# Y-Claw/Multilevel-GNN

Measured on AMD Instinct MI355X. Metric: graphs/sec fwd+bwd, 3-level GNN on 10k-node d=128 synthetic; HBM GB/s %peak, higher is better.
Workload: dtype f32; 1 GPU; configs[1]: ER graphs N=10000 E=160000 x64 per GPU, d=128, 3 GENConv(softmax, res+, LayerNorm) + projection pooling G=25000 k=2 + DiffPool 146->37->10, fp32; step = CSR build (of the next batch, on a second stream) + fwd + bwd + grad all-reduce + Adam; graphs_per_gpu=64, global_batch=64, parallelism=dp1, world_size=1, allreduce_bytes=1429768

## Files before the change

multilevel-gnn_amd/csrc/densesage.hip:

```cpp
#include "common.h"
#include "launch.h"
#include "mlgnn.h"
#include "tile_gemm.h"

namespace mlgnn {

constexpr int kDsMaxN = 160, kDsMaxC = 128, kDsMaxO = 64, kDsMaxNAdj = 48;
constexpr int kDsBlock = 1024, kDsWaves = kDsBlock / kWave;
constexpr int kDsSO = kDsMaxO + 1;
constexpr float kDsNormEps = 1e-12f;

struct DsArgs {
  const void* x; const void* adj; const void* w_rel; const void* w_root; const float* bias;
  const void* gy; const void* y; const float* rinv_in;
  void* y_out; float* rinv; void* gx; void* gadj; float* ws;
  int n; int C; int O; int adj_batched; int normalize; int ws_cols;
};

template <typename AB>
__device__ __forceinline__ void ds_degrees(const AB ab, int n, float* deg, float* raw) {
  const int lane = threadIdx.x & (kWave - 1), wave = threadIdx.x / kWave;
  for (int r = wave; r < n; r += kDsWaves) {
    float s = 0.f;
    for (int j = lane; j < n; j += kWave) s += ab[(size_t)r * n + j];
#pragma unroll
    for (int off = 32; off > 0; off >>= 1) s += __shfl_xor(s, off);
    if (lane == 0) {
      if (raw) raw[r] = s;
      deg[r] = fmaxf(s, 1.0f);
    }
  }
}

struct DsLds { int so, sx, np; };
__host__ __device__ inline DsLds ds_lds(int n, int C, int O) {
  DsLds l;
  l.np = (n + 15) & ~15;
  l.so = ((O + 15) & ~15) + 1;
  l.sx = C + 1 + (C & 1);
  return l;
}
inline size_t ds_fwd_lds_bytes(int n, int C, int O) {
  const DsLds l = ds_lds(n, C, O);
  return ((size_t)l.np * l.so + (size_t)l.np * l.sx + l.np) * 4;
}
inline size_t ds_bwd_lds_bytes(int n, int C, int O, bool adj_grad) {
  const DsLds l = ds_lds(n, C, O);
  size_t f = (size_t)2 * l.np * l.so + 2 * l.np;
  if (adj_grad) f += (size_t)l.np * l.so + (size_t)l.np * (l.np + 1);
  return f * 4;
}

template <typename T>
__global__ __launch_bounds__(kDsBlock) void dense_sage_fwd_kernel(const DsArgs p) {
  extern __shared__ __attribute__((aligned(16))) float ds_smem[];
  const int b = blockIdx.x, tid = threadIdx.x;
  const int lane = tid & (kWave - 1), wave = tid / kWave;
  const int n = p.n, C = p.C, O = p.O;
  const DsLds L = ds_lds(n, C, O);
  const int SO = L.so, SX = L.sx;
  float* Pm_ = ds_smem;
  float* Xm_ = Pm_ + (size_t)L.np * SO;
  float* deg = Xm_ + (size_t)L.np * SX;
#define P(r, c) Pm_[(r) * SO + (c)]
#define X(r, c) Xm_[(r) * SX + (c)]
  const StoredIn<T> xb{static_cast<const T*>(p.x) + (size_t)b * n * C};
  const StoredIn<T> ab{static_cast<const T*>(p.adj) + (p.adj_batched ? (size_t)b * n * n : 0)};
  const StoredIn<T> w_rel{static_cast<const T*>(p.w_rel)}, w_root{static_cast<const T*>(p.w_root)};
  const int NP = (n + 15) & ~15, OP = (O + 15) & ~15;
  const int Nt = NP / 16, Ot = OP / 16;
  const int l15 = lane & 15, lq = lane >> 4;

  ds_degrees(ab, n, deg, nullptr);
  for (int idx = tid; idx < NP * C; idx += kDsBlock) {
    const int r = idx / C, c = idx % C;
    X(r, c) = r < n ? xb[idx] : 0.f;
  }
  __syncthreads();
  for (int t = wave; t < Nt * Ot; t += kDsWaves) {
    const int i0 = (t / Ot) * 16, j0 = (t % Ot) * 16;
    const f32x4 acc = tile_gemm(C,
        [&](int i, int k) { return k < C ? X(i0 + i, k) : 0.f; },
        [&](int k, int j) { return (j0 + j < O && k < C) ? w_rel[(size_t)(j0 + j) * C + k] : 0.f; });
#pragma unroll
    for (int r = 0; r < 4; ++r) P(i0 + lq * 4 + r, j0 + l15) = acc[r];
  }
  __syncthreads();
  f32x4 keep[(kDsMaxN / 16) * (kDsMaxO / 16) / kDsWaves + 1];
  int nk = 0;
  for (int t = wave; t < Nt * Ot; t += kDsWaves, ++nk) {
    const int i0 = (t / Ot) * 16, j0 = (t % Ot) * 16;
    f32x4 acc = tile_gemm(n,
        [&](int i, int k) { return (i0 + i < n && k < n) ? ab[(size_t)(i0 + i) * n + k] : 0.f; },
        [&](int k, int j) { return k < n ? P(k, j0 + j) : 0.f; });
    const f32x4 root = tile_gemm(C,
        [&](int i, int k) { return k < C ? X(i0 + i, k) : 0.f; },
        [&](int k, int j) { return (j0 + j < O && k < C) ? w_root[(size_t)(j0 + j) * C + k] : 0.f; });
    const float bj = (p.bias && j0 + l15 < O) ? p.bias[j0 + l15] : 0.f;
#pragma unroll
    for (int r = 0; r < 4; ++r) {
      const int row = i0 + lq * 4 + r;
      acc[r] = acc[r] / deg[min(row, n - 1)] + root[r] + bj;
    }
    keep[nk] = acc;
  }
  __syncthreads();
  nk = 0;
  for (int t = wave; t < Nt * Ot; t += kDsWaves, ++nk) {
    const int i0 = (t / Ot) * 16, j0 = (t % Ot) * 16;
#pragma unroll
    for (int r = 0; r < 4; ++r) P(i0 + lq * 4 + r, j0 + l15) = keep[nk][r];
  }
  __syncthreads();
  for (int r = wave; r < n; r += kDsWaves) {
    const float v = lane < O ? P(r, lane) : 0.f;
    float ss = v * v;
#pragma unroll
    for (int off = 32; off > 0; off >>= 1) ss += __shfl_xor(ss, off);
    const float ri = p.normalize ? 1.0f / fmaxf(sqrtf(ss), kDsNormEps) : 1.0f;
    if (lane < O) stored_write<T>(p.y_out, ((size_t)b * n + r) * O + lane, v * ri);
    if (lane == 0) p.rinv[(size_t)b * n + r] = ri;
  }
}
#undef P
#undef X

template <typename T>
__global__ __launch_bounds__(kDsBlock) void dense_sage_bwd_kernel(const DsArgs p) {
  extern __shared__ __attribute__((aligned(16))) float ds_smem[];
  const int b = blockIdx.x, tid = threadIdx.x;
  const int lane = tid & (kWave - 1), wave = tid / kWave;
  const int n = p.n, C = p.C, O = p.O;
  const DsLds L = ds_lds(n, C, O);
  const int SO = L.so, SM = L.np + 1;
  float* G_ = ds_smem;
  float* GP_ = G_ + (size_t)L.np * SO;
  float* deg = GP_ + (size_t)L.np * SO;
  float* raw = deg + L.np;
  float* Pm_ = raw + L.np;
  float* M_ = Pm_ + (size_t)L.np * SO;
#define G(r, c) G_[(r) * SO + (c)]
#define GP(r, c) GP_[(r) * SO + (c)]
#define Pm(r, c) Pm_[(r) * SO + (c)]
#define M(r, c) M_[(r) * SM + (c)]
  const StoredIn<T> xb{static_cast<const T*>(p.x) + (size_t)b * n * C};
  const StoredIn<T> ab{static_cast<const T*>(p.adj) + (p.adj_batched ? (size_t)b * n * n : 0)};
  const StoredIn<T> w_rel{static_cast<const T*>(p.w_rel)}, w_root{static_cast<const T*>(p.w_root)};
  const StoredIn<T> gyb{static_cast<const T*>(p.gy) + (size_t)b * n * O};
  const StoredIn<T> yb{static_cast<const T*>(p.y) + (size_t)b * n * O};
  const int NP = (n + 15) & ~15, OP = (O + 15) & ~15, CP = (C + 15) & ~15;
  const int Nt = NP / 16, Ot = OP / 16, Ct = CP / 16;
  const int l15 = lane & 15, lq = lane >> 4;

  ds_degrees(ab, n, deg, raw);
  for (int r = wave; r < NP; r += kDsWaves) {
    float gv = 0.f, yv = 0.f;
    if (r < n && lane < O) { gv = gyb[(size_t)r * O + lane]; yv = yb[(size_t)r * O + lane]; }
    float dot = gv * yv;
#pragma unroll
    for (int off = 32; off > 0; off >>= 1) dot += __shfl_xor(dot, off);
    const float ri = r < n ? p.rinv_in[(size_t)b * n + r] : 0.f;
    const float g = p.normalize ? (gv - yv * dot) * ri : gv;
    if (lane < OP) G(r, lane) = (r < n && lane < O) ? g : 0.f;
  }
  __syncthreads();
  for (int t = wave; t < Nt * Ot; t += kDsWaves) {
    const int i0 = (t / Ot) * 16, j0 = (t % Ot) * 16;
    const f32x4 acc = tile_gemm(n,
        [&](int i, int k) { return (i0 + i < n && k < n) ? ab[(size_t)k * n + i0 + i] : 0.f; },
        [&](int k, int j) { return k < n ? G(k, j0 + j) / deg[k] : 0.f; });
#pragma unroll
    for (int r = 0; r < 4; ++r) GP(i0 + lq * 4 + r, j0 + l15) = acc[r];
  }
  __syncthreads();
  const size_t gx_off = (size_t)b * n * C;
  for (int t = wave; t < Nt * Ct; t += kDsWaves) {
    const int i0 = (t / Ct) * 16, c0 = (t % Ct) * 16;
    f32x4 acc = tile_gemm(O,
        [&](int i, int k) { return k < O ? GP(i0 + i, k) : 0.f; },
        [&](int k, int j) { return (k < O && c0 + j < C) ? w_rel[(size_t)k * C + c0 + j] : 0.f; });
    const f32x4 t2 = tile_gemm(O,
        [&](int i, int k) { return k < O ? G(i0 + i, k) : 0.f; },
        [&](int k, int j) { return (k < O && c0 + j < C) ? w_root[(size_t)k * C + c0 + j] : 0.f; });
#pragma unroll
    for (int r = 0; r < 4; ++r) {
      const int row = i0 + lq * 4 + r, col = c0 + l15;
      if (row < n && col < C) stored_write<T>(p.gx, gx_off + (size_t)row * C + col, acc[r] + t2[r]);
    }
  }
  float* wsb = p.ws + (size_t)b * p.ws_cols;
  for (int t = wave; t < 2 * Ot * Ct; t += kDsWaves) {
    const int which = t / (Ot * Ct), tt = t % (Ot * Ct);
    const int o0 = (tt / Ct) * 16, c0 = (tt % Ct) * 16;
    const float* src = which == 0 ? GP_ : G_;
    const f32x4 acc = tile_gemm(n,
        [&](int i, int k) { return k < n ? src[k * SO + o0 + i] : 0.f; },
        [&](int k, int j) { return (k < n && c0 + j < C) ? xb[(size_t)k * C + c0 + j] : 0.f; });
#pragma unroll
    for (int r = 0; r < 4; ++r) {
      const int o = o0 + lq * 4 + r, c = c0 + l15;
      if (o < O && c < C) wsb[(size_t)which * O * C + (size_t)o * C + c] = acc[r];
    }
  }
  for (int o = tid; o < O; o += kDsBlock) {
    float s = 0.f;
    for (int r = 0; r < n; ++r) s += G(r, o);
    wsb[(size_t)2 * O * C + o] = s;
  }
  if (p.gadj) {
    for (int t = wave; t < Nt * Ot; t += kDsWaves) {
      const int i0 = (t / Ot) * 16, j0 = (t % Ot) * 16;
      const f32x4 acc = tile_gemm(C,
          [&](int i, int k) { return (i0 + i < n && k < C) ? xb[(size_t)(i0 + i) * C + k] : 0.f; },
          [&](int k, int j) { return (j0 + j < O && k < C) ? w_rel[(size_t)(j0 + j) * C + k] : 0.f; });
#pragma unroll
      for (int r = 0; r < 4; ++r) Pm(i0 + lq * 4 + r, j0 + l15) = acc[r];
    }
    __syncthreads();
    for (int t = wave; t < Nt * Nt; t += kDsWaves) {
      const int i0 = (t / Nt) * 16, j0 = (t % Nt) * 16;
      const f32x4 acc = tile_gemm(O,
          [&](int i, int k) { return k < O ? G(i0 + i, k) : 0.f; },
          [&](int k, int j) { return k < O ? Pm(j0 + j, k) : 0.f; });
#pragma unroll
      for (int r = 0; r < 4; ++r) M(i0 + lq * 4 + r, j0 + l15) = acc[r];
    }
    __syncthreads();
    const size_t ga_off = (size_t)b * n * n;
    for (int r = wave; r < n; r += kDsWaves) {
      float c = lane < n ? ab[(size_t)r * n + lane] * M(r, lane) : 0.f;
#pragma unroll
      for (int off = 32; off > 0; off >>= 1) c += __shfl_xor(c, off);
      const float ci = raw[r] >= 1.0f ? c / deg[r] : 0.f;
      if (lane < n) stored_write<T>(p.gadj, ga_off + (size_t)r * n + lane, (M(r, lane) - ci) / deg[r]);
    }
  }
}
#undef G
#undef GP
#undef Pm
#undef M

static bool ds_dims_ok(int64_t n, int64_t C, int64_t O) {
  return n >= 1 && n <= kDsMaxN && C >= 1 && C <= kDsMaxC && O >= 1 && O <= kDsMaxO;
}

}

using namespace mlgnn;

extern "C" int mlgnn_dense_sage_supported(int64_t n, int64_t C, int64_t O, int need_grad_adj) {
  return (ds_dims_ok(n, C, O) && (!need_grad_adj || n <= kDsMaxNAdj)) ? 1 : 0;
}

extern "C" int64_t mlgnn_dense_sage_bwd_workspace_floats(int64_t B, int64_t C, int64_t O) {
  if (B < 0 || C <= 0 || O <= 0) return MLGNN_E_SHAPE;
  return B * (2 * O * C + O);
}

extern "C" int mlgnn_dense_sage_fwd(const void* x, const void* adj, const void* w_rel, const void* w_root,
                                    const float* bias, void* y, float* rinv, int64_t B, int64_t n, int64_t C,
                                    int64_t O, int adj_batched, int normalize, int dtype, void* stream) {
  if (dtype != MLGNN_DTYPE_F32 && dtype != MLGNN_DTYPE_BF16) return MLGNN_E_DTYPE;
  if (B < 0 || !ds_dims_ok(n, C, O)) return MLGNN_E_SHAPE;
  if (B == 0) return 0;
  if (!x || !adj || !w_rel || !w_root || !y || !rinv) return MLGNN_E_NULL;
  DsArgs a = {};
  a.x = x; a.adj = adj; a.w_rel = w_rel; a.w_root = w_root;
  a.bias = bias; a.y_out = y; a.rinv = rinv;
  a.n = (int)n; a.C = (int)C; a.O = (int)O; a.adj_batched = adj_batched; a.normalize = normalize;
  const size_t lds = ds_fwd_lds_bytes((int)n, (int)C, (int)O);
  static size_t fwd_attr = 0;
  if (lds > fwd_attr) {
    const int most = (int)ds_fwd_lds_bytes(kDsMaxN, kDsMaxC, kDsMaxO);
    if (const hipError_t e = allow_dynamic_lds(&dense_sage_fwd_kernel<float>, most); e != hipSuccess) return (int)e;
    if (const hipError_t e = allow_dynamic_lds(&dense_sage_fwd_kernel<bf16_t>, most); e != hipSuccess) return (int)e;
    fwd_attr = (size_t)most;
  }
  if (dtype == MLGNN_DTYPE_BF16) hipLaunchKernelGGL(dense_sage_fwd_kernel<bf16_t>, dim3((unsigned)B), dim3(kDsBlock), lds, (hipStream_t)stream, a);
  else hipLaunchKernelGGL(dense_sage_fwd_kernel<float>, dim3((unsigned)B), dim3(kDsBlock), lds, (hipStream_t)stream, a);
  return (int)hipGetLastError();
}

extern "C" int mlgnn_dense_sage_bwd(const void* grad_y, const void* y, const float* rinv, const void* x,
                                    const void* adj, const void* w_rel, const void* w_root, void* grad_x,
                                    void* grad_adj, float* grad_w, float* workspace, int64_t workspace_floats,
                                    int64_t B, int64_t n, int64_t C, int64_t O, int adj_batched, int normalize,
                                    int dtype, void* stream) {
  if (dtype != MLGNN_DTYPE_F32 && dtype != MLGNN_DTYPE_BF16) return MLGNN_E_DTYPE;
  if (B < 0 || !ds_dims_ok(n, C, O)) return MLGNN_E_SHAPE;
  if (grad_adj && n > kDsMaxNAdj) return MLGNN_E_SHAPE;
  if (!grad_w) return MLGNN_E_NULL;
  const int cols = (int)(2 * O * C + O);
  hipStream_t s = (hipStream_t)stream;
  if (B == 0) return (int)hipMemsetAsync(grad_w, 0, (size_t)cols * 4, s);
  if (!grad_y || !y || !rinv || !x || !adj || !w_rel || !w_root || !grad_x || !workspace) return MLGNN_E_NULL;
  if (workspace_floats < B * cols) return MLGNN_E_WORKSPACE;
  DsArgs a = {};
  a.x = x; a.adj = adj; a.w_rel = w_rel; a.w_root = w_root;
  a.gy = grad_y; a.y = y; a.rinv_in = rinv;
  a.gx = grad_x; a.gadj = grad_adj; a.ws = workspace; a.ws_cols = cols;
  a.n = (int)n; a.C = (int)C; a.O = (int)O; a.adj_batched = adj_batched; a.normalize = normalize;
  const size_t lds = ds_bwd_lds_bytes((int)n, (int)C, (int)O, grad_adj != nullptr);
  static size_t bwd_attr = 0;
  if (lds > bwd_attr) {
    const size_t most = ds_bwd_lds_bytes(kDsMaxN, kDsMaxC, kDsMaxO, false) > ds_bwd_lds_bytes(kDsMaxNAdj, kDsMaxC, kDsMaxO, true)
                            ? ds_bwd_lds_bytes(kDsMaxN, kDsMaxC, kDsMaxO, false) : ds_bwd_lds_bytes(kDsMaxNAdj, kDsMaxC, kDsMaxO, true);
    if (const hipError_t e = allow_dynamic_lds(&dense_sage_bwd_kernel<float>, (int)most); e != hipSuccess) return (int)e;
    if (const hipError_t e = allow_dynamic_lds(&dense_sage_bwd_kernel<bf16_t>, (int)most); e != hipSuccess) return (int)e;
    bwd_attr = most;
  }
  if (dtype == MLGNN_DTYPE_BF16) hipLaunchKernelGGL(dense_sage_bwd_kernel<bf16_t>, dim3((unsigned)B), dim3(kDsBlock), lds, s, a);
  else hipLaunchKernelGGL(dense_sage_bwd_kernel<float>, dim3((unsigned)B), dim3(kDsBlock), lds, s, a);
  int err = (int)hipGetLastError();
  if (err) return err;
  launch_reduce_partials(workspace, grad_w, (int)B, cols, s);
  return (int)hipGetLastError();
}
```

multilevel-gnn_amd/csrc/tile_gemm.h:

```cpp
#pragma once
#include "common.h"

namespace mlgnn {

using f32x4 = __attribute__((ext_vector_type(4))) float;

constexpr int kTileUnroll = 8;

template <typename FA, typename FB>
__device__ __forceinline__ f32x4 tile_gemm(int kdim, FA a_at, FB b_at) {
  const int lane = threadIdx.x & (kWave - 1);
  const int l15 = lane & 15, lk = lane >> 4;
  f32x4 acc = {0.f, 0.f, 0.f, 0.f};
  for (int k0 = 0; k0 < kdim; k0 += 4 * kTileUnroll) {
    float a[kTileUnroll], b[kTileUnroll];
#pragma unroll
    for (int u = 0; u < kTileUnroll; ++u) {
      a[u] = a_at(l15, k0 + 4 * u + lk);
      b[u] = b_at(k0 + 4 * u + lk, l15);
    }
#pragma unroll
    for (int u = 0; u < kTileUnroll; ++u) acc = __builtin_amdgcn_mfma_f32_16x16x4f32(a[u], b[u], acc, 0, 0, 0);
  }
  return acc;
}

}
```

Measured before the change: 5505 graphs/s.

## Stage DenseSAGE forward operands in LDS and keep weight fragments register-resident

The dense SAGE forward kernel now stages x, both weight matrices, and the adjacency into LDS using 16-byte vector loads where alignment allows, instead of reading weights and adjacency element-wise from global memory inside the MFMA loops. Each wave owns a fixed column tile and keeps its W_rel/W_root fragments in registers, computing the rel and root products for up to three row tiles in one pass. Degrees are then computed from the LDS copy of the adjacency, and the separate keep/write-back pass is merged into a single epilogue. This cuts redundant global traffic and strided scalar loads, at the cost of higher LDS usage, an extra sync inside the K-block loop, and more register pressure from the resident fragments.

```diff
diff --git a/multilevel-gnn_amd/csrc/densesage.hip b/multilevel-gnn_amd/csrc/densesage.hip
--- a/multilevel-gnn_amd/csrc/densesage.hip
+++ b/multilevel-gnn_amd/csrc/densesage.hip
@@ -7,22 +7,24 @@
 
 constexpr int kDsMaxN = 160, kDsMaxC = 128, kDsMaxO = 64, kDsMaxNAdj = 48;
 constexpr int kDsBlock = 1024, kDsWaves = kDsBlock / kWave;
-constexpr int kDsSO = kDsMaxO + 1;
 constexpr float kDsNormEps = 1e-12f;
+constexpr int kDsFwdTiles = 3;
+static_assert(kDsFwdTiles * (kDsWaves / (kDsMaxO / 16)) >= kDsMaxN / 16, "row tiles of one column tile per wave");
 
 struct DsArgs {
   const void* x; const void* adj; const void* w_rel; const void* w_root; const float* bias;
   const void* gy; const void* y; const float* rinv_in;
   void* y_out; float* rinv; void* gx; void* gadj; float* ws;
   int n; int C; int O; int adj_batched; int normalize; int ws_cols;
+  int vec16;
 };
 
 template <typename AB>
-__device__ __forceinline__ void ds_degrees(const AB ab, int n, float* deg, float* raw) {
+__device__ __forceinline__ void ds_degrees(const AB ab, int n, int stride, float* deg, float* raw) {
   const int lane = threadIdx.x & (kWave - 1), wave = threadIdx.x / kWave;
   for (int r = wave; r < n; r += kDsWaves) {
     float s = 0.f;
-    for (int j = lane; j < n; j += kWave) s += ab[(size_t)r * n + j];
+    for (int j = lane; j < n; j += kWave) s += ab[(size_t)r * stride + j];
 #pragma unroll
     for (int off = 32; off > 0; off >>= 1) s += __shfl_xor(s, off);
     if (lane == 0) {
@@ -32,23 +34,64 @@
   }
 }
 
-struct DsLds { int so, sx, np; };
+struct DsLds { int so, sx, sa, np, op; };
 __host__ __device__ inline DsLds ds_lds(int n, int C, int O) {
   DsLds l;
   l.np = (n + 15) & ~15;
-  l.so = ((O + 15) & ~15) + 1;
-  l.sx = C + 1 + (C & 1);
+  l.op = (O + 15) & ~15;
+  l.so = l.op + 1;
+  l.sx = ((C + 31) & ~31) + 1;
+  l.sa = ((n + 31) & ~31) + 1;
   return l;
+}
+__host__ __device__ inline int ds_fwd_floats(const DsLds& l) {
+  const int first = l.np * l.sx + 2 * l.op * l.sx, then = l.np * (l.sx > l.sa ? l.sx : l.sa) + l.np * l.so;
+  return first > then ? first : then;
 }
 inline size_t ds_fwd_lds_bytes(int n, int C, int O) {
   const DsLds l = ds_lds(n, C, O);
-  return ((size_t)l.np * l.so + (size_t)l.np * l.sx + l.np) * 4;
+  return ((size_t)ds_fwd_floats(l) + l.np) * 4;
 }
 inline size_t ds_bwd_lds_bytes(int n, int C, int O, bool adj_grad) {
   const DsLds l = ds_lds(n, C, O);
   size_t f = (size_t)2 * l.np * l.so + 2 * l.np;
   if (adj_grad) f += (size_t)l.np * l.so + (size_t)l.np * (l.np + 1);
   return f * 4;
+}
+
+template <typename T, int V>
+__device__ __forceinline__ void ds_stage_run(float* img, int stride, const T* src, int cols, int first, int count) {
+  const int step = V * kDsBlock, dr = step / cols, dc = step - dr * cols;
+  int e = first + V * (int)threadIdx.x;
+  int r = e / cols, c = e - r * cols;
+  for (int i = threadIdx.x; i < count; i += kDsBlock, e += step) {
+    float v[V];
+    load_t<T, V>(v, src + e);
+    int rr = r, cc = c;
+#pragma unroll
+    for (int q = 0; q < V; ++q) {
+      img[rr * stride + cc] = v[q];
+      if (++cc == cols) { cc = 0; ++rr; }
+    }
+    c += dc; r += dr;
+    if (c >= cols) { c -= cols; ++r; }
+  }
+}
+
+template <typename T>
+__device__ __forceinline__ void ds_stage(float* img, int stride, const T* src, int rows, int cols, int rows_p,
+                                         int cols_p, int vec16) {
+  constexpr int V = 16 / (int)sizeof(T);
+  const int lane = threadIdx.x & (kWave - 1), wave = threadIdx.x / kWave;
+  const int total = rows * cols;
+  int head = total;
+  if (vec16) head = min(total, (int)(((0 - reinterpret_cast<uintptr_t>(src)) & 15) / sizeof(T)));
+  const int nvec = (total - head) / V;
+  ds_stage_run<T, 1>(img, stride, src, cols, 0, head);
+  if (nvec > 0) ds_stage_run<T, V>(img, stride, src, cols, head, nvec);
+  ds_stage_run<T, 1>(img, stride, src, cols, head + V * nvec, total - head - V * nvec);
+  for (int r = wave; r < rows_p; r += kDsWaves)
+    for (int c = (r < rows ? cols : 0) + lane; c < cols_p; c += kWave) img[r * stride + c] = 0.f;
 }
 
 template <typename T>
@@ -58,58 +101,79 @@
   const int lane = tid & (kWave - 1), wave = tid / kWave;
   const int n = p.n, C = p.C, O = p.O;
   const DsLds L = ds_lds(n, C, O);
-  const int SO = L.so, SX = L.sx;
-  float* Pm_ = ds_smem;
-  float* Xm_ = Pm_ + (size_t)L.np * SO;
-  float* deg = Xm_ + (size_t)L.np * SX;
+  const int SO = L.so, SX = L.sx, SA = L.sa;
+  float* Xm_ = ds_smem;
+  float* Wr_ = Xm_ + (size_t)L.np * SX;
+  float* Wt_ = Wr_ + (size_t)L.op * SX;
+  float* Am_ = Xm_;
+  float* deg = ds_smem + ds_fwd_floats(L);
+  float* Pm_ = deg - (size_t)L.np * SO;
 #define P(r, c) Pm_[(r) * SO + (c)]
 #define X(r, c) Xm_[(r) * SX + (c)]
-  const StoredIn<T> xb{static_cast<const T*>(p.x) + (size_t)b * n * C};
-  const StoredIn<T> ab{static_cast<const T*>(p.adj) + (p.adj_batched ? (size_t)b * n * n : 0)};
-  const StoredIn<T> w_rel{static_cast<const T*>(p.w_rel)}, w_root{static_cast<const T*>(p.w_root)};
+#define A(r, c) Am_[(r) * SA + (c)]
+  const T* xg = static_cast<const T*>(p.x) + (size_t)b * n * C;
+  const T* ag = static_cast<const T*>(p.adj) + (p.adj_batched ? (size_t)b * n * n : 0);
   const int NP = (n + 15) & ~15, OP = (O + 15) & ~15;
   const int Nt = NP / 16, Ot = OP / 16;
   const int l15 = lane & 15, lq = lane >> 4;
-
-  ds_degrees(ab, n, deg, nullptr);
-  for (int idx = tid; idx < NP * C; idx += kDsBlock) {
-    const int r = idx / C, c = idx % C;
-    X(r, c) = r < n ? xb[idx] : 0.f;
-  }
-  __syncthreads();
-  for (int t = wave; t < Nt * Ot; t += kDsWaves) {
-    const int i0 = (t / Ot) * 16, j0 = (t % Ot) * 16;
-    const f32x4 acc = tile_gemm(C,
-        [&](int i, int k) { return k < C ? X(i0 + i, k) : 0.f; },
-        [&](int k, int j) { return (j0 + j < O && k < C) ? w_rel[(size_t)(j0 + j) * C + k] : 0.f; });
-#pragma unroll
-    for (int r = 0; r < 4; ++r) P(i0 + lq * 4 + r, j0 + l15) = acc[r];
-  }
-  __syncthreads();
-  f32x4 keep[(kDsMaxN / 16) * (kDsMaxO / 16) / kDsWaves + 1];
-  int nk = 0;
-  for (int t = wave; t < Nt * Ot; t += kDsWaves, ++nk) {
-    const int i0 = (t / Ot) * 16, j0 = (t % Ot) * 16;
-    f32x4 acc = tile_gemm(n,
-        [&](int i, int k) { return (i0 + i < n && k < n) ? ab[(size_t)(i0 + i) * n + k] : 0.f; },
-        [&](int k, int j) { return k < n ? P(k, j0 + j) : 0.f; });
-    const f32x4 root = tile_gemm(C,
-        [&](int i, int k) { return k < C ? X(i0 + i, k) : 0.f; },
-        [&](int k, int j) { return (j0 + j < O && k < C) ? w_root[(size_t)(j0 + j) * C + k] : 0.f; });
+  const int wpc = kDsWaves / Ot, j0 = (wave % Ot) * 16, first = wave / Ot;
+  const bool active = first < wpc;
+
+  ds_stage<T>(Xm_, SX, xg, n, C, NP, SX - 1, p.vec16);
+  ds_stage<T>(Wr_, SX, static_cast<const T*>(p.w_rel), O, C, OP, SX - 1, p.vec16);
+  ds_stage<T>(Wt_, SX, static_cast<const T*>(p.w_root), O, C, OP, SX - 1, p.vec16);
+  __syncthreads();
+  f32x4 keep[kDsFwdTiles];
+  for_k_blocks<kDsMaxC / 32>((C + 31) >> 5, [&](auto kb) {
+    constexpr int KB = decltype(kb)::value;
+    float wr[8 * KB], wt[8 * KB];
+    if (active) {
+      frag_load<KB>(wr, [&](int k) { return Wr_[(j0 + l15) * SX + k]; });
+      frag_load<KB>(wt, [&](int k) { return Wt_[(j0 + l15) * SX + k]; });
+    }
+    __syncthreads();
+    if (active) {
+#pragma unroll
+      for (int s = 0; s < kDsFwdTiles; ++s) {
+        const int i0 = (first + s * wpc) * 16;
+        if (i0 < NP) {
+          f32x4 acc;
+          tile_gemm2_b_resident<KB>(wr, wt, [&](int i, int k) { return X(i0 + i, k); }, acc, keep[s]);
+#pragma unroll
+          for (int r = 0; r < 4; ++r) P(i0 + lq * 4 + r, j0 + l15) = acc[r];
+        }
+      }
+    }
+  });
+  __syncthreads();
+  ds_stage<T>(Am_, SA, ag, n, n, NP, (n + 31) & ~31, p.vec16);
+  __syncthreads();
+  ds_degrees(Am_, n, SA, deg, nullptr);
+  f32x4 agg[kDsFwdTiles];
+  if (active) {
+#pragma unroll
+    for (int s = 0; s < kDsFwdTiles; ++s) {
+      const int i0 = (first + s * wpc) * 16;
+      if (i0 < NP)
+        agg[s] = tile_gemm(n,
+            [&](int i, int k) { return A(i0 + i, k); },
+            [&](int k, int j) { return k < n ? P(k, j0 + j) : 0.f; });
+    }
+  }
+  __syncthreads();
+  if (active) {
     const float bj = (p.bias && j0 + l15 < O) ? p.bias[j0 + l15] : 0.f;
 #pragma unroll
-    for (int r = 0; r < 4; ++r) {
-      const int row = i0 + lq * 4 + r;
-      acc[r] = acc[r] / deg[min(row, n - 1)] + root[r] + bj;
-    }
-    keep[nk] = acc;
-  }
-  __syncthreads();
-  nk = 0;
-  for (int t = wave; t < Nt * Ot; t += kDsWaves, ++nk) {
-    const int i0 = (t / Ot) * 16, j0 = (t % Ot) * 16;
-#pragma unroll
-    for (int r = 0; r < 4; ++r) P(i0 + lq * 4 + r, j0 + l15) = keep[nk][r];
+    for (int s = 0; s < kDsFwdTiles; ++s) {
+      const int i0 = (first + s * wpc) * 16;
+      if (i0 < NP) {
+#pragma unroll
+        for (int r = 0; r < 4; ++r) {
+          const int row = i0 + lq * 4 + r;
+          P(row, j0 + l15) = agg[s][r] / deg[min(row, n - 1)] + keep[s][r] + bj;
+        }
+      }
+    }
   }
   __syncthreads();
   for (int r = wave; r < n; r += kDsWaves) {
@@ -124,6 +188,7 @@
 }
 #undef P
 #undef X
+#undef A
 
 template <typename T>
 __global__ __launch_bounds__(kDsBlock) void dense_sage_bwd_kernel(const DsArgs p) {
@@ -152,7 +217,7 @@
   const int Nt = NP / 16, Ot = OP / 16, Ct = CP / 16;
   const int l15 = lane & 15, lq = lane >> 4;
 
-  ds_degrees(ab, n, deg, raw);
+  ds_degrees(ab, n, n, deg, raw);
   for (int r = wave; r < NP; r += kDsWaves) {
     float gv = 0.f, yv = 0.f;
     if (r < n && lane < O) { gv = gyb[(size_t)r * O + lane]; yv = yb[(size_t)r * O + lane]; }
@@ -269,6 +334,7 @@
   a.x = x; a.adj = adj; a.w_rel = w_rel; a.w_root = w_root;
   a.bias = bias; a.y_out = y; a.rinv = rinv;
   a.n = (int)n; a.C = (int)C; a.O = (int)O; a.adj_batched = adj_batched; a.normalize = normalize;
+  a.vec16 = aligned<16>(x, adj, w_rel, w_root) ? 1 : 0;
   const size_t lds = ds_fwd_lds_bytes((int)n, (int)C, (int)O);
   static size_t fwd_attr = 0;
   if (lds > fwd_attr) {
diff --git a/multilevel-gnn_amd/csrc/tile_gemm.h b/multilevel-gnn_amd/csrc/tile_gemm.h
--- a/multilevel-gnn_amd/csrc/tile_gemm.h
+++ b/multilevel-gnn_amd/csrc/tile_gemm.h
@@ -1,5 +1,6 @@
 #pragma once
 #include "common.h"
+#include "dispatch.h"
 
 namespace mlgnn {
 
@@ -25,4 +26,39 @@
   return acc;
 }
 
+template <int KB, typename F>
+__device__ __forceinline__ void frag_load(float (&f)[8 * KB], F at) {
+  const int lk = (threadIdx.x & (kWave - 1)) >> 4;
+#pragma unroll
+  for (int u = 0; u < 8 * KB; ++u) f[u] = at(4 * u + lk);
 }
+
+template <int KB, typename FA>
+__device__ __forceinline__ void tile_gemm2_b_resident(const float (&b0)[8 * KB], const float (&b1)[8 * KB], FA a_at,
+                                                      f32x4& acc0, f32x4& acc1) {
+  const int lane = threadIdx.x & (kWave - 1);
+  const int l15 = lane & 15, lk = lane >> 4;
+  acc0 = f32x4{0.f, 0.f, 0.f, 0.f};
+  acc1 = f32x4{0.f, 0.f, 0.f, 0.f};
+#pragma unroll
+  for (int blk = 0; blk < KB; ++blk) {
+    float a[kTileUnroll];
+#pragma unroll
+    for (int u = 0; u < kTileUnroll; ++u) a[u] = a_at(l15, 32 * blk + 4 * u + lk);
+#pragma unroll
+    for (int u = 0; u < kTileUnroll; ++u) {
+      acc0 = __builtin_amdgcn_mfma_f32_16x16x4f32(a[u], b0[8 * blk + u], acc0, 0, 0, 0);
+      acc1 = __builtin_amdgcn_mfma_f32_16x16x4f32(a[u], b1[8 * blk + u], acc1, 0, 0, 0);
+    }
+  }
+}
+
+template <int MAXKB, typename F>
+__device__ __forceinline__ void for_k_blocks(int kb, F&& f) {
+  if constexpr (MAXKB > 1) {
+    if (kb < MAXKB) { for_k_blocks<MAXKB - 1>(kb, f); return; }
+  }
+  f(IC<MAXKB>{});
+}
+
+}
```

Result: faster. 5561 graphs/s (median of 6 runs) (+1.0%).
